# SMLC-NYSBC/TARGET-VAE

Measured on AMD Instinct MI355X. Metric: training images/sec (fwd+bwd+Adam), P8 z=2 64x64 bs=256/GPU, higher is better.
Workload: dtype f32 (matrix products: operands as TWO fp16 parts under one power-of-two scale PER ROW of the operand (row / column of the product), 3 fp16 MFMAs per product block -- 2 where one operand is the exact 0 / 1 matrix -- fp32 accumulate: at least as accurate against fp64 as the fp32 matrix pipe (profiles/

## Files before the change

### include/tvae_hip.h

```cpp
#ifndef TVAE_HIP_H
#define TVAE_HIP_H
#ifdef __cplusplus
extern "C" {
#endif

typedef void* tvae_stream_t;

int tvae_abi_version(void);


int tvae_rotate_bank_fwd(const float* weight, const int* tap_idx, const float* tap_w, float* bank, int C, int Cin,
                         int ksz, int R, tvae_stream_t stream);
int tvae_rotate_bank_bwd(const float* dbank, const int* csr_ptr, const int* csr_r, const int* csr_dst,
                         const float* csr_w, float* dweight, int C, int Cin, int ksz, int R, int accumulate,
                         tvae_stream_t stream);

int tvae_conv1_fwd(const float* y, const float* bank, const float* bias, float* out, int B, int Cin, int n, int ksz,
                   int pad, int C, int R, int act, float slope, tvae_stream_t stream);
int tvae_conv1_wgrad(const float* y, const float* dpre, float* dbank, float* ws, long ws_floats, int B, int Cin,
                     int n, int ksz, int pad, int C, int R, tvae_stream_t stream);

int tvae_linear_fwd(const float* W, const float* X, const float* bias, const float* gbias, int group,
                    const float* res, float* Y, int M, int N, int K, long ldx, long ldy, int act, float slope,
                    tvae_stream_t stream);
// ... 32 lines not shown
                       long ws_floats, int B, int Cin, int n, int ksz, int pad, int C, int R, int act, float slope,
                       int parts, tvae_stream_t stream);
int tvae_conv1_wgrad_dft(const float* dpre, const float* at, float* dbank, float* dbias, float* ws, long ws_floats, int B,
                         int Cin, int n, int ksz, int pad, int C, int R, int parts, tvae_stream_t stream);

long tvae_dense_x6_bytes(int rows, int K);
int tvae_dense_split3(const float* W, long ldw, void* a3, long a3_bytes, int rows, int K, int transpose,
                      const float* scale, float* rowsum, tvae_stream_t stream);
int tvae_dense_split2h(const float* W, long ldw, void* a3, long a3_bytes, int rows, int K, int transpose,
                       const float* scale, float* rowsum, tvae_stream_t stream);
int tvae_linear_fwd_x6(const void* w3, const float* X, const float* bias, const float* res, float* Y, int M, int N,
                       int K, long ldx, long ldy, int act, float slope, const float* col_w, const float* col_b,
                       float* col_y, const float* va_xr, const float* va_wc, const float* va_bc, const float* va_lb,
                       int va_np, void* sign_bits, int parts, const float* x_amax, float* y_amax, tvae_stream_t stream);
int tvae_linear_dgrad_x6(const void* w3t, const float* dpre, const float* add, const float* aux, float* dX, int M,
                         int N, int K, long ldd, long ldx, int mask, float slope, const float* in_xr,
                         const float* in_wc, float* in_gxr, float* in_part, long in_part_floats, const float* vg_wo,
                         const float* vg_gy, const float* vg_csum, const float* in_bc, const float* in_lb, int in_np,
                         float* rs_part, long rs_part_floats, const float* rs_wo, const float* rs_gysum, float* rs_db,
                         float* rs_dwo, int parts, const void* vg_bits, const float* rs_rowdot, const float* rs_bias,
                         const float* x_amax, float* y_amax, tvae_stream_t stream);
int tvae_dgrad_rowsum_total(const float* rs_part, int ntiles, int M, const float* rs_wo, const float* rs_gysum, float slope,
                            float* rs_db, float* rs_dwo, const float* rs_rowdot, const float* rs_bias, tvae_stream_t stream);
int tvae_dec_in_total(float* part, int B, int cpi, int F, float* Simg, float* dbc, float* dWc, tvae_stream_t stream);
long tvae_linear_wgrad_x6_ws_floats(int M, int N, int K);
int tvae_linear_wgrad_x6(const float* dpre, const float* X, float* dW, float* ws, long ws_floats, int M, int N, int K,
                         long ldd, long ldx, int accumulate, const float* vg_wo, const float* vg_gy, int vg_act,
                         float vg_slope, const float* va_xr, const float* va_wc, const float* va_bc, const float* va_lb,
                         int va_np, const void* vg_bits, int parts, const float* rd_w, long rd_ldw, float* rd_rowdot,
                         const float* a_amax, const float* x_amax, int x_amax_rows, tvae_stream_t stream);

int tvae_dec_out_bwd(const float* gy, int n_out, const float* Wo, const float* H, long ldh, float* D, long ldd, int F,
                     long N, int act, float slope, float* part, long part_floats, float* tot, tvae_stream_t stream);
int tvae_dec_in_bwd(const float* d, long ldd, const float* xr, const float* Wc, int F, int B, int Np, float* gxr,
                    float* Simg, float* dbc, float* dWc, float* part, long part_floats, tvae_stream_t stream);
int tvae_heads_fwd(const float* W, const float* X, long ldx, const float* bias, float* Y, long ldy, int nh, int C,
                   long N, tvae_stream_t stream);
int tvae_heads_bwd(const float* W, const float* dY, long ldy, const float* X, long ldx, float* dX, long lddx, int nh,
                   int C, long N, int act, float slope, float* part, long part_floats, float* tot,
                   tvae_stream_t stream);

int tvae_attn_head_fwd(const float* heads, long ldh, const float* E, const float* eps_z, const float* eps_t,
                       const float* p_r, const float* off, const float* p_tr, const float* grid, int B, int R, int P,
                       int zd, float sigma_p, float theta_off_scale, float* attn, float* q, float* a, float* z,
                       float* theta, float* dx, float* kl, float* part, long part_floats, tvae_stream_t stream);
int tvae_attn_head_bwd(const float* heads, long ldh, const float* q, const float* a, const float* eps_z,
// ... 75 lines not shown
```

### profiles/kernel_bench.py

```python
import os, sys, time
ROOT = os.path.dirname(os.path.dirname(os.path.abspath(__file__)))
sys.path[:0] = [ROOT, os.path.join(ROOT, 'target-vae_amd')]
import torch
import tvae._lib as _L
if os.environ.get('TVAE_LIB'):
    _L.LIB_PATH = os.path.abspath(os.environ['TVAE_LIB'])
from tvae._lib import call, set_gemm_mode, query
set_gemm_mode(os.environ.get('MODE', 'f32'))
print('mode', os.environ.get('MODE', 'f32'))
dev = torch.device('cuda:0')
reps = int(os.environ.get('REPS', '5'))
PARTS = int(os.environ.get('PARTS', '3'))
B = int(os.environ.get('B', '256'))
only = os.environ.get('ONLY', '')


def timeit(name, flops, fn):
    if only and not any(tok in name for tok in only.split(',')):
        return
    fn(); torch.cuda.synchronize()
    s, e = torch.cuda.Event(True), torch.cuda.Event(True)
    s.record()
    for _ in range(reps):
        fn()
# ... 83 lines not shown
    gxr = torch.empty(Nt, 2, device=dev); partf = torch.empty((Nt // 128) * F_ * 3, device=dev)
    wo1 = torch.randn(F_, device=dev); gy1 = torch.randn(Nt, device=dev)
    fl = 2.0 * F_ * F_ * Nt
    timeit('tail_dgrad_plain', fl, lambda: call('tvae_linear_dgrad_x6', w3t, h1, None, h3, h2, F_, Nt, F_, Nt, Nt, 1, 0.01, None, None, None, None, 0, None, None, None, None, None, 0, None, 0, None, None, None, None, PARTS))
    timeit('tail_dgrad_intail', fl, lambda: call('tvae_linear_dgrad_x6', w3t, h1, None, h3, None, F_, Nt, F_, Nt, Nt, 1, 0.01, xr2, wc2, gxr, partf, partf.numel(), None, None, None, None, None, 0, None, 0, None, None, None, None, PARTS))
    timeit('tail_dgrad_virt', fl, lambda: call('tvae_linear_dgrad_x6', w3t, h1, None, h3, h2, F_, Nt, F_, Nt, Nt, 1, 0.01, None, None, None, None, 0, wo1, gy1, None, None, None, 0, None, 0, None, None, None, None, PARTS))
    timeit('tail_dgrad_both', fl, lambda: call('tvae_linear_dgrad_x6', w3t, h1, None, h3, None, F_, Nt, F_, Nt, Nt, 1, 0.01, xr2, wc2, gxr, partf, partf.numel(), wo1, gy1, None, None, None, 0, None, 0, None, None, None, None, PARTS))
    timeit('tail_wgrad_plain', fl, lambda: call('tvae_linear_wgrad_x6', h1, h3, dW, ws, ws.numel(), F_, Nt, F_, Nt, Nt, 0, None, None, 0, 0.01, None, None, None, None, 0, None, PARTS))
    Np_ = n * n
    bc2 = torch.randn(F_, device=dev); lb2 = torch.randn(B, F_, device=dev)
    va = (xr2, wc2, bc2, lb2, Np_)
    cy = torch.empty(Nt, device=dev)
    timeit('tail_fwd_step', fl, lambda: call('tvae_linear_fwd_x6', w3, None, bb, None, h2, F_, Nt, F_, Nt, Nt, 1, 0.01, wo1, bb[:1].contiguous(), cy, *va, None, PARTS))
    sb = torch.zeros(F_, Nt // 32, dtype=torch.int32, device=dev)
    timeit('tail_fwd_step+bits', fl, lambda: call('tvae_linear_fwd_x6', w3, None, bb, None, h2, F_, Nt, F_, Nt, Nt, 1, 0.01, wo1, bb[:1].contiguous(), cy, *va, sb, PARTS))
    timeit('tail_fwd_step_nostore', fl, lambda: call('tvae_linear_fwd_x6', w3, None, bb, None, None, F_, Nt, F_, Nt, Nt, 1, 0.01, wo1, bb[:1].contiguous(), cy, *va, None, PARTS))
    csum2 = torch.empty(F_, device=dev)
    w3s = torch.empty_like(w3)
    call('tvae_dense_split3', W, F_, w3s, w3s.numel() * 4, F_, F_, 1, wo1, csum2)
    timeit('tail_dgrad_step', fl, lambda: call('tvae_linear_dgrad_x6', w3s, h1, None, None, None, F_, Nt, F_, Nt, Nt, 1, 0.01, xr2, wc2, gxr, partf, partf.numel(), None, gy1, csum2, bc2, lb2, Np_, None, 0, None, None, None, None, PARTS))
    timeit('tail_dgrad_generic', fl, lambda: call('tvae_linear_dgrad_x6', w3t, h1, None, None, None, F_, Nt, F_, Nt, Nt, 1, 0.01, xr2, wc2, gxr, partf, partf.numel(), wo1, gy1, None, bc2, lb2, Np_, None, 0, None, None, None, None, PARTS))
    hbits = torch.zeros(F_, Nt // 32, dtype=torch.int32, device=dev).random_(-2 ** 31, 2 ** 31 - 1)
    timeit('tail_wgrad_step', fl, lambda: call('tvae_linear_wgrad_x6', None, None, dW, ws, ws.numel(), F_, Nt, F_, Nt, Nt, 0, wo1, gy1, 1, 0.01, *va, hbits, PARTS))
    timeit('tail_wgrad_from_H', fl, lambda: call('tvae_linear_wgrad_x6', h1, None, dW, ws, ws.numel(), F_, Nt, F_, Nt, Nt, 0, wo1, gy1, 1, 0.01, *va, None, PARTS))
    timeit('tail_wgrad_virt', fl, lambda: call('tvae_linear_wgrad_x6', h1, h3, dW, ws, ws.numel(), F_, Nt, F_, Nt, Nt, 0, wo1, gy1, 1, 0.01, None, None, None, None, 0, None, PARTS))
if only and 'enc' in only:
    nh = 7
    Wh = torch.randn(nh, C, device=dev) * 0.1
    bh = torch.randn(nh, device=dev)
    heads = torch.empty(nh, N, device=dev)
    A1.normal_()
    fl2 = 2.0 * C * C * N
    timeit('enc_conv2_fwd_f32', fl2, lambda: call('tvae_linear_fwd', W2, A1, b2, None, 1, None, H, C, N, C, N, N, 1, 0.01))
    timeit('enc_heads_fwd', 2.0 * nh * C * N, lambda: call('tvae_heads_fwd', Wh, H, N, bh, heads, N, nh, C, N))
    w23 = torch.empty(query('tvae_dense_x6_bytes', C, C) // 4, device=dev)
    call('tvae_dense_split3', W2, C, w23, w23.numel() * 4, C, C, 0, None, None)
    H2 = torch.empty(C, N, device=dev)
    heads2 = torch.empty(nh, N, device=dev)
    timeit('enc_tail_fwd_x6', fl2, lambda: call('tvae_enc_tail_fwd_x6', w23, A1, N, b2, Wh, bh, nh, H2, N, heads2, N, None, None, C, N, 1, 0.01, PARTS))
    bits = torch.zeros(2, N, 4, dtype=torch.int32, device=dev)
    timeit('enc_tail_fwd_x6+bits', fl2, lambda: call('tvae_enc_tail_fwd_x6', w23, A1, N, b2, Wh, bh, nh, H2, N, heads2, N, bits[0], bits[1], C, N, 1, 0.01, PARTS))
    print('fused fwd vs separate: H %.3e heads %.3e' % (float((H2 - H).norm() / H.norm()), float((heads2 - heads).norm() / heads.norm())))
    dheads = torch.randn(nh, N, device=dev)
    dH = torch.empty(C, N, device=dev)
    npan = (N + 511) // 512
    part = torch.empty(npan * C * (nh + 1), device=dev)
# ... 14 lines not shown
```

### target-vae_amd/csrc/abi_dense_x6.hip

```cpp
#include "abi_dense_x6.hpp"
#include "dense_prepass_kernels.hpp"

using namespace tvae;

namespace {
struct Dx6Instance {
    int xv, epi, parts;
    int (*launch)(TVAE_DX6_LAUNCH_ARGS);
};
const Dx6Instance DX6_INSTANCES[] = {
#define TVAE_DX6(XV_, E_, NP_) {XV_, E_, NP_, dense_x6_launch<XV_, E_, NP_>},
#include "dense_x6_instances.def"
#undef TVAE_DX6
};
int dense_x6_dispatch(int xv, int epi, int parts, TVAE_DX6_LAUNCH_ARGS) {
    for (const Dx6Instance& i : DX6_INSTANCES)
        if (i.xv == xv && i.epi == epi && i.parts == parts)
            return i.launch(a3, X, ldx, ep, M, Mpad, N, K, K8pad, tm, bt, cd, it, vg, va, st, hs);
    return (int)hipErrorInvalidValue;
}
}

namespace tvae {
int h3_zero_slots(float* p, int n, int threads, hipStream_t st) {
// ... 78 lines not shown
    *rc = (int)hipGetLastError();
    return true;
}
}

namespace {
__global__ void dgrad_rowsum_total_kernel(const float* __restrict__ part, int ntiles, int K, const float* __restrict__ wo,
                                          const float* __restrict__ gysum, float slope, float* __restrict__ db,
                                          float* __restrict__ dwo, const float* __restrict__ rowdot,
                                          const float* __restrict__ bias) {
    __shared__ float sm[2 * 16];
    const int m = blockIdx.x;
    float s[2] = {0.f, 0.f};
    for (int t = threadIdx.x; t < ntiles; t += blockDim.x) {
        const float2 v = *reinterpret_cast<const float2*>(part + ((long)m * ntiles + t) * 2);
        s[0] += v.x;
        if (!rowdot) s[1] += v.y;
    }
    block_sum<2>(s, sm);
    if (threadIdx.x == 0) {
        const float g0 = __fmaf_rn(1.f - slope, s[0], slope * gysum[0]);
        db[m] = wo[m] * g0;
        dwo[m] = rowdot ? __fmaf_rn(bias ? bias[m] : 0.f, g0, rowdot[m]) : s[1];
    }
}
}

extern "C" {

long tvae_dense_x6_bytes(int rows, int K) { return dense_x6_bytes(rows, K); }
static int dense_split(const float* W, long ldw, void* a3, long a3_bytes, int rows, int K, int transpose,
                       const float* scale, float* rowsum, int parts, tvae_stream_t stream) {
    if (rows <= 0 || K <= 0) return 0;
    if (a3_bytes < tvae_dense_x6_bytes(rows, K) || !aligned16(a3)) return (int)hipErrorInvalidValue;
    const int Rpad = x6_round_up(rows, DX6_ROWS), K8pad = dense_k8pad(K);
    const long total = (long)K8pad * Rpad;
    if (parts == 2) {
        float* tr = h3_trailer(a3, rows, K);
        if (transpose)
            hipLaunchKernelGGL(dense_rowmax_kernel, dim3(Rpad / 64), dim3(1024), 0, S(stream), W, ldw, rows, Rpad, K, transpose,
                               scale, tr);
        else
            hipLaunchKernelGGL(dense_rowmax_rows_kernel, dim3(Rpad / 4), dim3(256), 0, S(stream), W, ldw, rows, Rpad, K, scale, tr);
        TVAE_CHECK_LAUNCH();
        const int rc = dense_split2h(W, ldw, (uint4*)a3, rows, Rpad, K, K8pad, transpose, scale, tr, S(stream));
        if (rc) return rc;
// ... 112 lines not shown
    if (in_xr) {
        if (!in_wc || !in_gxr || !in_part || in_part_floats < (long)(N / 128) * K * 3) return (int)hipErrorInvalidValue;
    } else if (!dX) {
        return (int)hipErrorInvalidValue;
    }
    if (vg_bits && !(vg_csum && rs_part && (rs_rowdot || !rs_db) && N % 32 == 0))
        return (int)hipErrorInvalidValue;
    if (rs_rowdot && !vg_bits) return (int)hipErrorInvalidValue;
    if (rs_part) {
        if (!vg_csum || !vg_gy || !rs_wo || !rs_gysum || (!rs_db != !rs_dwo) || M > DX6_ROWS || N % 128 != 0 ||
            rs_part_floats < (long)(N / 128) * M * 2 || (reinterpret_cast<size_t>(rs_part) & 7))
            return (int)hipErrorInvalidValue;
    }
    int rc = launch_dense_x6(w3t, dpre, ldd, ep, K, N, M, parts, S(stream), ColDot{nullptr, nullptr, nullptr},
                             InTail{in_xr, in_wc, in_gxr, in_part, in_bc, in_lb, in_np > 0 ? in_np : 1},
                             VirtGrad{vg_wo, vg_gy, mask, slope, vg_csum, (const unsigned*)vg_bits, rs_part, 0},
                             VirtAct{nullptr, nullptr, nullptr, nullptr, 1, 0, 0.f}, x_amax);
    if (rc || !rs_part || !rs_db || N <= 0 || K <= 0) return rc;
    hipLaunchKernelGGL(dgrad_rowsum_total_kernel, dim3(M), dim3(256), 0, S(stream), (const float*)rs_part, N / 128, M, rs_wo,
                       rs_gysum, slope, rs_db, rs_dwo, rs_rowdot, rs_bias);
    TVAE_CHECK_LAUNCH();
    return 0;
}
int tvae_dgrad_rowsum_total(const float* rs_part, int ntiles, int M, const float* rs_wo, const float* rs_gysum, float slope,
                            float* rs_db, float* rs_dwo, const float* rs_rowdot, const float* rs_bias, tvae_stream_t stream) {
    if (!rs_part || !rs_wo || !rs_gysum || !rs_db || !rs_dwo || ntiles <= 0 || M <= 0) return (int)hipErrorInvalidValue;
    hipLaunchKernelGGL(dgrad_rowsum_total_kernel, dim3(M), dim3(256), 0, S(stream), rs_part, ntiles, M, rs_wo, rs_gysum, slope,
                       rs_db, rs_dwo, rs_rowdot, rs_bias);
    TVAE_CHECK_LAUNCH();
    return 0;
}


}
```

### target-vae_amd/csrc/abi_dense_x6.hpp

```cpp
#pragma once
#include "abi_common.hpp"
#include "dense_x6_kernels.hpp"

namespace tvae {

static inline int dense_k8pad(int K) { return x6_round_up((K + 7) / 8, 2); }
static inline long dense_x6_bytes(int rows, int K) {
    const long Rpad = x6_round_up(rows, DX6_ROWS), K8pad = dense_k8pad(K);
    return 3 * K8pad * Rpad * 16;
}

static inline bool dense_x6_xres_fits(int rows_per_problem, int Mb, int N, int K, int parts) {
    const int nk = dense_k8pad(K) / 2;
    const size_t lds = (size_t)nk * parts * 256 * 16 + (size_t)(Mb + 128) * 4;
    return (parts == 2 || parts == 3) && (nk == 12 || nk == 10 || nk == 8) && N % 128 == 0 && rows_per_problem % DX6_ROWS == 0 &&
           Mb >= rows_per_problem && lds <= X6_LDS_MAX;
}

static inline float* h3_trailer(const void* a3, int rows, int K) {
    const long total = (long)dense_k8pad(K) * x6_round_up(rows, DX6_ROWS);
    return reinterpret_cast<float*>(const_cast<void*>(a3)) + 2 * total * 4;
}

#define TVAE_DX6_LAUNCH_ARGS                                                                                          \
    const uint4 *a3, const float *X, long ldx, const Epilogue &ep, int M, int Mpad, int N, int K, int K8pad,          \
        const TileMap &tm, const DenseBatch &bt, const ColDot &cd, const InTail &it, const VirtGrad &vg,              \
        const VirtAct &va, hipStream_t st, const H3Scale &hs
template <int XV, int EPI, int NP>
TVAE_INTERNAL int dense_x6_launch(TVAE_DX6_LAUNCH_ARGS);

#define TVAE_WG_LAUNCH_ARGS                                                                                           \
    int variant, const float *dY, long ldd, const float *X, long ldx, float *ws, int M, int Kf, int N, int nchunk,     \
        const TileMap &tm, const DenseBatch &bt, long dy_stride, const VirtGrad &vg, const VirtAct &va,               \
        const ATile &atile, hipStream_t st, const H3Scale &hs
TVAE_INTERNAL int dense_wgrad_x6_launch_p3(TVAE_WG_LAUNCH_ARGS);
TVAE_INTERNAL int dense_wgrad_x6_launch_p2(TVAE_WG_LAUNCH_ARGS);
TVAE_INTERNAL int dense_wgrad_x6_launch_p1(TVAE_WG_LAUNCH_ARGS);
TVAE_INTERNAL int dense_wgrad_x6_launch_p1_abf(TVAE_WG_LAUNCH_ARGS);

#define TVAE_WGW_LAUNCH_ARGS                                                                                          \
    const float *dY, long ldd, const float *X, long ldx, float *ws, int M, int Kf, int N, int nchunk, const TileMap &tm, \
        const DenseBatch &bt, long dy_stride, const ATile &atile, hipStream_t st, const H3Scale &hs
TVAE_INTERNAL int dense_wgrad_x6_wide_p3(TVAE_WGW_LAUNCH_ARGS);
TVAE_INTERNAL int dense_wgrad_x6_wide_p2(TVAE_WGW_LAUNCH_ARGS);

TVAE_INTERNAL int h3_zero_slots(float* p, int n, int threads, hipStream_t st);
TVAE_INTERNAL int dense_split2h(const float* W, long ldw, uint4* a3, int rows, int Rpad, int K, int K8pad, int transpose,
                                const float* scale, const float* rowmax, hipStream_t st);
TVAE_INTERNAL int dec_l0_bound(const float* xr, int N, const float* wc, const float* bc, const float* lb, long nlb, int K,
                               float* slots, hipStream_t st);

TVAE_INTERNAL int dense_x6_batched4(const void* w3, const float* X, long ldx, const Epilogue& ep, int rows_per_problem,
// ... 15 lines not shown
```

### target-vae_amd/csrc/dense_x6_kernels.hpp

```cpp
#pragma once
#include <hip/hip_runtime.h>
#include <type_traits>
#include "conv_x6_device.hpp"
#include "small_device.hpp"

#ifndef TVAE_ABL
#define TVAE_ABL 0
#endif

namespace tvae {

template <int NP>
__device__ __forceinline__ void mfma_np(f32x16& acc, const Cell16 (&a)[3], const Cell16 (&b)[3]) {
    if (NP == 3) mfma6(acc, a, b);
    else if (NP == 2) mfma3h(acc, a, b);
    else acc = __builtin_amdgcn_mfma_f32_32x32x16_bf16(a[0].v, b[0].v, acc, 0, 0, 0);
}
template <int NP>
__device__ __forceinline__ void mfma_part(f32x16& acc, const Cell16& a, const Cell16& b) {
    if (NP == 2) acc = __builtin_amdgcn_mfma_f32_32x32x16_f16(a.h, b.h, acc, 0, 0, 0);
    else acc = __builtin_amdgcn_mfma_f32_32x32x16_bf16(a.v, b.v, acc, 0, 0, 0);
}
template <int NP> struct OneBits { static constexpr unsigned lo = NP == 2 ? 0x3c00u : 0x3f80u, hi = lo << 16; };
template <bool XS>
// ... 204 lines not shown
#pragma unroll
                for (int j = 0; j < 4; ++j) {
                    float v = NP == 2 ? __fmaf_rn(acc[i][j][r] * ixv[j], aq[p], bq[p]) : acc[i][j][r] + bq[p];
                    v = fmaxf(v, v * slope);
                    ysum[j] = __fmaf_rn(wq[p], v, ysum[j]);
                    const unsigned long long bl = __ballot(v > 0.f);
                    sw[j] = (unsigned)(half ? bl >> 32 : bl);
                }
                if ((lane & 31) == 0 && sbits)
                    *reinterpret_cast<uint4*>(sbits + (long)(m0 + rb + p) * bitw + (n0 >> 5)) = make_uint4(sw[0], sw[1], sw[2], sw[3]);
            }
            __builtin_amdgcn_sched_barrier(0);
        }
}

__device__ __forceinline__ float half_wave_sum_hi(float x) {
    x = dpp_add<0xB1>(x);
    x = dpp_add<0x4E>(x);
    x = dpp_add<0x141>(x);
    x = dpp_add<0x140>(x);
    return x + __int_as_float(__builtin_amdgcn_update_dpp(0, __float_as_int(x), 0x142, 0xA, 0xF, false));
}

template <int NP>
__device__ __forceinline__ void dense_x6_epilogue_lean_in(f32x16 (&acc)[2][4], const float* bsm, const float* wc2,
                                                          const float* cbm, const float* h3a, float slope, float oms, int wave,
                                                          int lane, int m0, int M, int tile_n, const float (&gyv)[4],
                                                          const float (&x0)[4], const float (&x1)[4], float* part,
                                                          float (&gsum)[4][2]) {
    float gx0[4], gx1[4];
#pragma unroll
    for (int j = 0; j < 4; ++j) {
        gx0[j] = gyv[j] * x0[j];
        gx1[j] = gyv[j] * x1[j];
    }
    const int half = lane >> 5;
#pragma unroll
    for (int i = 0; i < 2; ++i)
#pragma unroll
        for (int q = 0; q < 4; ++q) {
            const int rb = wave * 64 + i * 32 + 8 * q + 4 * half;
            const float4 b4 = *reinterpret_cast<const float4*>(bsm + rb);
            const float4 c4 = *reinterpret_cast<const float4*>(cbm + rb);
            const float4 l4 = *reinterpret_cast<const float4*>(cbm + DX6_ROWS + rb);
            const float4 wA = *reinterpret_cast<const float4*>(wc2 + 2 * rb), wB = *reinterpret_cast<const float4*>(wc2 + 2 * rb + 4);
            float4 a4 = make_float4(1.f, 1.f, 1.f, 1.f);
            if (NP == 2) a4 = *reinterpret_cast<const float4*>(h3a + rb);
            const float bq[4] = {b4.x, b4.y, b4.z, b4.w}, cq[4] = {c4.x, c4.y, c4.z, c4.w}, lq[4] = {l4.x, l4.y, l4.z, l4.w};
            const float aq[4] = {a4.x, a4.y, a4.z, a4.w};
            const float w0q[4] = {wA.x, wA.z, wB.x, wB.z}, w1q[4] = {wA.y, wA.w, wB.y, wB.w};
#pragma unroll
            for (int p = 0; p < 4; ++p) {
                const int r = 4 * q + p;
                float rs0 = 0.f, rs1 = 0.f, rs2 = 0.f;
#pragma unroll
                for (int j = 0; j < 4; ++j) {
                    const float t = __fmaf_rn(oms, NP == 2 ? acc[i][j][r] * aq[p] : acc[i][j][r], bq[p]);
                    const float pre = dec_l0_pre(w0q[p], w1q[p], cq[p], lq[p], x0[j], x1[j]);
                    const float u = pre > 0.f ? t : t * slope;
                    rs0 = __fmaf_rn(u, gyv[j], rs0);
                    rs1 = __fmaf_rn(u, gx0[j], rs1);
                    rs2 = __fmaf_rn(u, gx1[j], rs2);
                    gsum[j][0] = __fmaf_rn(w0q[p], u, gsum[j][0]);
                    gsum[j][1] = __fmaf_rn(w1q[p], u, gsum[j][1]);
                }
                rs0 = half_wave_sum_hi(rs0);
                rs1 = half_wave_sum_hi(rs1);
// ... 1380 lines not shown
```

### target-vae_amd/tvae/_lib.py

```python
from __future__ import annotations

import ctypes
import os

import torch

_HERE = os.path.dirname(os.path.abspath(__file__))
LIB_PATH = os.environ.get('TVAE_LIB') or os.path.join(os.path.dirname(_HERE), 'csrc', 'build', 'libtvae_hip.so')

SIGNATURES = {
    'tvae_rotate_bank_fwd': 'ppppiiii',
    'tvae_rotate_bank_bwd': 'ppppppiiiii',
    'tvae_conv1_fwd': 'ppppiiiiiiiif',
    'tvae_conv1_wgrad': 'ppppl iiiiiii'.replace(' ', ''),
    'tvae_bank_split3': 'ppliiii',
    'tvae_conv1_fwd_x6': 'ppppiiiiiiiif',
    'tvae_dy_split3': 'ppliiiiiii',
    'tvae_conv1_wgrad_x6': 'ppppliiiiiii',
    'tvae_conv1_fwd_dft': 'ppppppliiiiiiiifi',
    'tvae_conv1_wgrad_dft': 'pppppliiiiiiii',
    'tvae_dense_split3': 'plpliiipp',
    'tvae_dense_split2h': 'plpliiipp',
    'tvae_linear_fwd_x6': 'pppppiiillifpppppppipipp',
    'tvae_linear_dgrad_x6': 'pppppiiillifpppplpppppiplppppippppp',
    'tvae_dec_in_total': 'piiippp',
    'tvae_dgrad_rowsum_total': 'piippfpppp',
    'tvae_linear_wgrad_x6': 'ppppliiillippifppppipiplpppi',
    'tvae_linear_fwd': 'ppppippiiillif',
    'tvae_linear_dgrad': 'pppppiiillif',
    'tvae_linear_wgrad': 'ppppliiilli',
    'tvae_rowdot_seg': 'plpiiiipp',
    'tvae_seg_sum': 'pilpfi',
    'tvae_coldot': 'pliipiipip',
    'tvae_outer_mask': 'pipiiplpliiif',
    'tvae_act_bwd': 'ppplif',
    'tvae_dec_out_bwd': 'pipplplilifplp',
    'tvae_dec_in_bwd': 'plppiiipppppl',
    'tvae_heads_fwd': 'pplppliil',
    'tvae_heads_bwd': 'pplplpliilifplp',
    'tvae_attn_head_fwd': 'plpppppppiiiiffppppppppl',
    'tvae_attn_head_bwd': 'plppppppppiiiiffpppppppppl',
    'tvae_get_latent': 'plpppiiiifppp',
    'tvae_enc_tail_fwd_x6': 'pplpppiplplppilifip',
    'tvae_enc_tail_dgrad_x6': 'ppplippplilfi',
    'tvae_enc_tail_wgrad_x6': 'plplipppplilfip',
    'tvae_enc_tail_fwd_wide': 'ppplppiplplppilifip',
    'tvae_enc_tail_dgrad_wide': 'ppplippplplilfip',
# ... 11 lines not shown
    'tvae_loglik_bwd': 'ppppiii',
    'tvae_elbo_reduce': 'ppippp',
    'tvae_elbo_reduce_bwd': 'pppipp',
    'tvae_ctf_corr': 'pppiiii',
    'tvae_loglik_masked_fwd': 'pppffiip',
    'tvae_loglik_masked_bwd': 'pppffiipp',
    'tvae_adam_flat': 'pppplfffffff',
}

QUERIES = {
    'tvae_conv1_x6_supported': ('iiii', 'i'),
    'tvae_conv1_x6_bank_bytes': ('iiii', 'l'),
    'tvae_conv1_x6_dy_bytes': ('iiiiii', 'l'),
    'tvae_dense_x6_bytes': ('ii', 'l'),
    'tvae_conv1_dft_supported': ('iiiiiii', 'i'),
    'tvae_conv1_dft_at_floats': ('iiiiiii', 'l'),
    'tvae_conv1_dft_ws_floats': ('iiiiiii', 'l'),
    'tvae_conv1_dft_frame': ('iiiiiii', 'i'),
    'tvae_conv1_dft_ring': ('iiiiiii', 'i'),
    'tvae_conv1_dft_route': ('iiiiiiiii', 'i'),
    'tvae_enc_tail_wgrad_x6_ws_floats': ('l', 'l'),
    'tvae_enc_tail_wide_max_rows': ('', 'i'),
    'tvae_linear_wgrad_x6_ws_floats': ('iii', 'l'),
}

OPTIONAL_TAIL = {'tvae_linear_wgrad_x6': 6}

_CT = {'p': ctypes.c_void_p, 'i': ctypes.c_int, 'l': ctypes.c_long, 'f': ctypes.c_float}
_lib = None


class TvaeHipError(RuntimeError):
    pass


def lib():
    global _lib
    if _lib is None:
        if not os.path.exists(LIB_PATH):
            raise TvaeHipError(
                f'{LIB_PATH} not found: build it with `make -C target-vae_amd/csrc` '
                '(or __graft_entry__.build()).  There is no CPU fallback.')
        L = ctypes.CDLL(LIB_PATH)
        for name, sig in SIGNATURES.items():
            fn = getattr(L, name)
            fn.restype = ctypes.c_int
# ... 198 lines not shown
```

### target-vae_amd/tvae/ops.py

```python
from __future__ import annotations

import math
import os
from typing import NamedTuple, Optional

import numpy as np
import torch

from . import tables
from ._lib import arithmetic, call, get_gemm_mode, parts, query, split_pipe

ACT_NONE, ACT_LRELU, ACT_TANH = 0, 1, 2
LRELU_SLOPE = 0.01


def _expect(cond: bool, what: str) -> None:
    if not cond:
        raise ValueError('tvae.ops: ' + what)


def act_code(activation) -> int:
    import torch.nn as nn
    a = activation() if isinstance(activation, type) else activation
    if isinstance(a, nn.LeakyReLU):
# ... 688 lines not shown

    @staticmethod
    def forward(ctx, xc, dx, theta):
        B, Np = theta.shape[0], xc.shape[0]
        _expect(tuple(xc.shape) == (Np, 2) and tuple(dx.shape) == (B, 2) and theta.dim() == 1, 'coordinate shapes')
        xc, dx, theta = xc.contiguous(), dx.contiguous(), theta.contiguous()
        xr = torch.empty(B, Np, 2, dtype=torch.float32, device=xc.device)
        call('tvae_coord_fwd', xc, dx, theta, xr, B, Np)
        ctx.save_for_backward(xc, dx, theta)
        return xr

    @staticmethod
    def backward(ctx, g):
        xc, dx, theta = ctx.saved_tensors
        B, Np = theta.shape[0], xc.shape[0]
        gdx = torch.empty(B, 2, dtype=torch.float32, device=xc.device)
        gth = torch.empty(B, dtype=torch.float32, device=xc.device)
        call('tvae_coord_bwd', xc, dx, theta, g.contiguous(), gdx, gth, B, Np)
        return None, gdx, gth


DEC_PAD = os.environ.get('TVAE_DEC_PAD', '1') != '0'
DEC_LD_PAD = int(os.environ.get('TVAE_DEC_LD_PAD', '64'))


class DecoderRoute(NamedTuple):
    ldn: int
    split: bool
    four_x6: bool
    four_dgrad_x6: bool
    virt_act: bool
    fused_out: bool
    virt_grad: bool
    sign_bits: bool
    no_h: bool
    h3: bool
    infer: bool


def decoder_route(B: int, Np: int, F_: int, n_hidden: int, n_out: int, act: int, resid: bool, Ff: int,
                  infer: bool) -> DecoderRoute:
    Nt = B * Np
    split = _dense_x6_ok(F_, Nt)
    virt_grad = n_hidden >= 1 and n_out == 1 and not resid and split
    sign_bits = virt_grad and act == ACT_LRELU
    ld_pad = DEC_LD_PAD and (Ff or n_hidden >= 2) and Nt % 16384 == 0 and split
# ... 197 lines not shown
                xb = xb * gy_amax()
            wg = _wgrad(dsrc, hprev, F_, Nt, F_, vg if use_vg else None, va, act, sbits, rowdot_w=W if from_bits else None,
                        a_amax=d_bnd if plain_h3 else None, x_amax=xb, ld=ldn)
            dW, rowdot = wg if from_bits else (wg, None)
            db = drow if drow is not None else _rowsum(d, F_, Nt, ld=ldn)
            drow = None
            fuse_in = li == 0 and rt.virt_act
            dprev = None if fuse_in else torch.empty(F_, ldn, dtype=torch.float32, device=dev)
            if rt.split:
                two_val = use_vg and act == ACT_LRELU
                p_d = 2 if (rt.h3 and (two_val or (not use_vg and d_bnd is not None))) else _p3()
                if p_d == 2 and not two_val:
                    _note('dec.dgrad_h3_meas')
                emit = dmeas[li:li + 1] if (dmeas is not None and not fuse_in) else None
                if two_val:
                    w3t, csum = _split_weight(W, F_, F_, True, 'x6_dense_wt', scale=vg[0], nparts=p_d)
                    _note('dec.virt_grad_2val')
                else:
                    w3t, csum = _split_weight(W, F_, F_, True, 'x6_dense_wt', nparts=p_d), None
                if fuse_in:
                    gxr_f = torch.empty(B, Np, 2, dtype=torch.float32, device=dev)
                    part_f = workspace(dev, (Nt // 128) * F_ * 3)
                rs_part = _scratch(dev, 'dec_rs_part', (Nt // 128) * F_ * 2) if from_bits else None
                with _timed('tvae_linear_dgrad_x6', p_d, two_val):
                    call('tvae_linear_dgrad_x6', w3t, dsrc, d if resid else None, hprev, dprev, F_, Nt, F_, ldn, ldn, act,
                         LRELU_SLOPE, xr.view(Nt, 2) if fuse_in else None, Wc.contiguous() if fuse_in else None,
                         gxr_f if fuse_in else None, part_f if fuse_in else None, part_f.numel() if fuse_in else 0,
                         vg[0] if (use_vg and not two_val) else None, vg[1] if use_vg else None, csum,
                         bc if va else None, LB if va else None, Np if va else 0,
                         rs_part, rs_part.numel() if from_bits else 0, vg[0] if from_bits else None,
                         dbo if from_bits else None, tot[0] if from_bits else None, tot[1] if from_bits else None, p_d,
                         sbits if from_bits else None, rowdot, b if from_bits else None,
                         d_bnd if (p_d == 2 and not two_val) else None, emit)
                if fuse_in:
                    _note('dec.fuse_in')
                d_bnd = emit
                if two_val and li == 0 and has_f and rt.h3:
                    d_bnd = gy_amax() * (W.detach().abs() * vg[0].detach().abs()[:, None]).sum(0).amax().reshape(1)
            else:
                call('tvae_linear_dgrad', W.contiguous(), d, d if resid else None, hprev, dprev, F_, Nt, F_, ldn, ldn,
                     act, LRELU_SLOPE)
            d = dprev
            grads_hidden.append((dW, db))
        grads_hidden.reverse()
        Simg = torch.empty(B, F_, dtype=torch.float32, device=dev)
        dbc = torch.empty(F_, dtype=torch.float32, device=dev)
        gxr = gxr_f if rt.virt_act else torch.empty(B, Np, 2, dtype=torch.float32, device=dev)
        if rt.virt_act:
            dWc = torch.empty(F_, 2, dtype=torch.float32, device=dev)
            call('tvae_dec_in_total', part_f, B, Np // 128, F_, Simg, dbc, dWc)
        elif has_f:
            call('tvae_rowdot_seg', d, ldn, None, 1, F_, Nt, Np, Simg)
            call('tvae_seg_sum', Simg, B, F_, dbc, 1.0, 0)
        else:
            dWc = torch.empty(F_, 2, dtype=torch.float32, device=dev)
            part = workspace(dev, B * ((Np + 1023) // 1024) * F_ * 3)
# ... 142 lines not shown
```

Baseline: 27940.

## Add half-row-tile dgrad kernel for fused decoder input layer with 2-part weights

Adds a specialized dgrad kernel for the decoder's first hidden layer when the virtual-gradient is two-valued and rebuilt from sign bits. Each block covers 256 of the 512 rows instead of the full height, which doubles the grid and raises the occupancy target to two blocks per CU. The partial input-gradient sums go to a 5-slot workspace, and a new total kernel reduces them alongside the row-sum bias/weight reduction. The cost is an extra workspace round trip and a narrow route that only fires for F=512 without residual connections.

```diff
diff --git a/include/tvae_hip.h b/include/tvae_hip.h
--- a/include/tvae_hip.h
+++ b/include/tvae_hip.h
@@ -78,6 +78,13 @@
                          const float* x_amax, float* y_amax, tvae_stream_t stream);
 int tvae_dgrad_rowsum_total(const float* rs_part, int ntiles, int M, const float* rs_wo, const float* rs_gysum, float slope,
                             float* rs_db, float* rs_dwo, const float* rs_rowdot, const float* rs_bias, tvae_stream_t stream);
+long tvae_linear_dgrad_x6_half_ws_floats(int N);
+int tvae_linear_dgrad_x6_half(const void* w3t, int M, int N, int K, float slope, const float* in_xr, const float* in_wc,
+                              float* in_gxr, float* in_part, long in_part_floats, const float* vg_gy, const float* vg_csum,
+                              const float* in_bc, const float* in_lb, int in_np, float* rs_part, long rs_part_floats,
+                              const float* rs_wo, const float* rs_gysum, float* rs_db, float* rs_dwo, int parts,
+                              const void* vg_bits, const float* rs_rowdot, const float* rs_bias, float* gws, long gws_floats,
+                              tvae_stream_t stream);
 int tvae_dec_in_total(float* part, int B, int cpi, int F, float* Simg, float* dbc, float* dWc, tvae_stream_t stream);
 long tvae_linear_wgrad_x6_ws_floats(int M, int N, int K);
 int tvae_linear_wgrad_x6(const float* dpre, const float* X, float* dW, float* ws, long ws_floats, int M, int N, int K,
diff --git a/profiles/kernel_bench.py b/profiles/kernel_bench.py
--- a/profiles/kernel_bench.py
+++ b/profiles/kernel_bench.py
@@ -129,6 +129,17 @@
     timeit('tail_dgrad_generic', fl, lambda: call('tvae_linear_dgrad_x6', w3t, h1, None, None, None, F_, Nt, F_, Nt, Nt, 1, 0.01, xr2, wc2, gxr, partf, partf.numel(), wo1, gy1, None, bc2, lb2, Np_, None, 0, None, None, None, None, PARTS))
     hbits = torch.zeros(F_, Nt // 32, dtype=torch.int32, device=dev).random_(-2 ** 31, 2 ** 31 - 1)
     timeit('tail_wgrad_step', fl, lambda: call('tvae_linear_wgrad_x6', None, None, dW, ws, ws.numel(), F_, Nt, F_, Nt, Nt, 0, wo1, gy1, 1, 0.01, *va, hbits, PARTS))
+    if PARTS == 2:
+        from tvae.ops import DGRAD_HALF
+        w3h = torch.empty_like(w3)
+        call('tvae_dense_split2h', W, F_, w3h, w3h.numel() * 4, F_, F_, 1, wo1, csum2)
+        rsp = torch.empty((Nt // 128) * F_ * 2, device=dev); gys = gy1.sum().reshape(1)
+        rdb, rdwo, rdot = torch.empty(F_, device=dev), torch.empty(F_, device=dev), torch.randn(F_, device=dev)
+        if DGRAD_HALF:
+            gws = torch.empty(query('tvae_linear_dgrad_x6_half_ws_floats', Nt), device=dev)
+            timeit('tail_dgrad_step_bits_half', fl, lambda: call('tvae_linear_dgrad_x6_half', w3h, F_, Nt, F_, 0.01, xr2, wc2, gxr, partf, partf.numel(), gy1, csum2, bc2, lb2, Np_, rsp, rsp.numel(), wo1, gys, rdb, rdwo, 2, hbits, rdot, bb, gws, gws.numel()))
+        else:
+            timeit('tail_dgrad_step_bits', fl, lambda: call('tvae_linear_dgrad_x6', w3h, None, None, None, None, F_, Nt, F_, Nt, Nt, 1, 0.01, xr2, wc2, gxr, partf, partf.numel(), None, gy1, csum2, bc2, lb2, Np_, rsp, rsp.numel(), wo1, gys, rdb, rdwo, 2, hbits, rdot, bb))
     timeit('tail_wgrad_from_H', fl, lambda: call('tvae_linear_wgrad_x6', h1, None, dW, ws, ws.numel(), F_, Nt, F_, Nt, Nt, 0, wo1, gy1, 1, 0.01, *va, None, PARTS))
     timeit('tail_wgrad_virt', fl, lambda: call('tvae_linear_wgrad_x6', h1, h3, dW, ws, ws.numel(), F_, Nt, F_, Nt, Nt, 0, wo1, gy1, 1, 0.01, None, None, None, None, 0, None, PARTS))
 if only and 'enc' in only:
diff --git a/target-vae_amd/csrc/abi_dense_x6.hip b/target-vae_amd/csrc/abi_dense_x6.hip
--- a/target-vae_amd/csrc/abi_dense_x6.hip
+++ b/target-vae_amd/csrc/abi_dense_x6.hip
@@ -1,5 +1,6 @@
 #include "abi_dense_x6.hpp"
 #include "dense_prepass_kernels.hpp"
+#include "dense_x6_half_shape.hpp"
 
 using namespace tvae;
 
@@ -124,6 +125,37 @@
         const float g0 = __fmaf_rn(1.f - slope, s[0], slope * gysum[0]);
         db[m] = wo[m] * g0;
         dwo[m] = rowdot ? __fmaf_rn(bias ? bias[m] : 0.f, g0, rowdot[m]) : s[1];
+    }
+}
+__global__ void dgrad_half_total_kernel(const float* __restrict__ part, int ntiles, int M, const float* __restrict__ wo,
+                                        const float* __restrict__ gysum, float slope, float* __restrict__ db,
+                                        float* __restrict__ dwo, const float* __restrict__ rowdot,
+                                        const float* __restrict__ bias, const float4* __restrict__ gws,
+                                        float4* __restrict__ gxr, long n4) {
+    __shared__ float sm[16];
+    if ((int)blockIdx.x >= M) {
+        const long i = (long)(blockIdx.x - M) * blockDim.x + threadIdx.x;
+        if (i >= n4) return;
+        float4 g = gws[i];
+#pragma unroll
+        for (int w = 1; w < 5; ++w) {
+            const float4 c = gws[w * n4 + i];
+            g.x += c.x;
+            g.y += c.y;
+            g.z += c.z;
+            g.w += c.w;
+        }
+        gxr[i] = g;
+        return;
+    }
+    const int m = blockIdx.x;
+    float s[1] = {0.f};
+    for (int t = threadIdx.x; t < ntiles; t += blockDim.x) s[0] += part[((long)m * ntiles + t) * 2];
+    block_sum<1>(s, sm);
+    if (threadIdx.x == 0) {
+        const float g0 = __fmaf_rn(1.f - slope, s[0], slope * gysum[0]);
+        db[m] = wo[m] * g0;
+        dwo[m] = __fmaf_rn(bias ? bias[m] : 0.f, g0, rowdot[m]);
     }
 }
 }
@@ -282,6 +314,40 @@
     TVAE_CHECK_LAUNCH();
     return 0;
 }
+long tvae_linear_dgrad_x6_half_ws_floats(int N) { return N > 0 ? (long)DXH_GWS_SLOTS * 2 * N : 0; }
+int tvae_linear_dgrad_x6_half(const void* w3t, int M, int N, int K, float slope, const float* in_xr, const float* in_wc,
+                              float* in_gxr, float* in_part, long in_part_floats, const float* vg_gy, const float* vg_csum,
+                              const float* in_bc, const float* in_lb, int in_np, float* rs_part, long rs_part_floats,
+                              const float* rs_wo, const float* rs_gysum, float* rs_db, float* rs_dwo, int parts,
+                              const void* vg_bits, const float* rs_rowdot, const float* rs_bias, float* gws, long gws_floats,
+                              tvae_stream_t stream) {
+    if (K != DX6_ROWS || M <= 0 || M > DXH_KMAX || N <= 0 || N % 128 != 0 || parts != 2 || in_np <= 0 || in_np % 128 != 0)
+        return (int)hipErrorInvalidValue;
+    if (!w3t || !in_xr || !in_wc || !in_gxr || !in_part || !vg_gy || !vg_csum || !in_bc || !rs_part || !rs_wo || !rs_gysum ||
+        !rs_db || !rs_dwo || !vg_bits || !rs_rowdot || !gws)
+        return (int)hipErrorInvalidValue;
+    if (in_part_floats < (long)(N / 128) * K * 3 || rs_part_floats < (long)(N / 128) * M * 2 ||
+        gws_floats < tvae_linear_dgrad_x6_half_ws_floats(N))
+        return (int)hipErrorInvalidValue;
+    if (!aligned16(w3t) || !aligned16(vg_bits) || !aligned16(gws) || !aligned16(in_gxr) || (reinterpret_cast<size_t>(rs_part) & 7))
+        return (int)hipErrorInvalidValue;
+    TileMap tm{DX6_ROWS / DXH_ROWS, N / 128, 1};
+    tm.pack = 1;
+    H3Scale hs = H3_NONE;
+    hs.amax_a = h3_trailer(w3t, K, M);
+    hs.a_rows = 1;
+    int rc = dense_x6_half_launch_p2((const uint4*)w3t, slope, K, DX6_ROWS, N, M, dense_k8pad(M), tm,
+                                     InTail{in_xr, in_wc, in_gxr, in_part, in_bc, in_lb, in_np},
+                                     VirtGrad{nullptr, vg_gy, ACT_LRELU, slope, vg_csum, (const unsigned*)vg_bits, rs_part, 0}, hs,
+                                     gws, S(stream));
+    if (rc) return rc;
+    const long n4 = (long)N / 2;
+    hipLaunchKernelGGL(dgrad_half_total_kernel, dim3((unsigned)(M + (n4 + 255) / 256)), dim3(256), 0, S(stream),
+                       (const float*)rs_part, N / 128, M, rs_wo, rs_gysum, slope, rs_db, rs_dwo, rs_rowdot, rs_bias,
+                       (const float4*)gws, (float4*)in_gxr, n4);
+    TVAE_CHECK_LAUNCH();
+    return 0;
+}
 int tvae_dgrad_rowsum_total(const float* rs_part, int ntiles, int M, const float* rs_wo, const float* rs_gysum, float slope,
                             float* rs_db, float* rs_dwo, const float* rs_rowdot, const float* rs_bias, tvae_stream_t stream) {
     if (!rs_part || !rs_wo || !rs_gysum || !rs_db || !rs_dwo || ntiles <= 0 || M <= 0) return (int)hipErrorInvalidValue;
diff --git a/target-vae_amd/csrc/abi_dense_x6.hpp b/target-vae_amd/csrc/abi_dense_x6.hpp
--- a/target-vae_amd/csrc/abi_dense_x6.hpp
+++ b/target-vae_amd/csrc/abi_dense_x6.hpp
@@ -28,6 +28,11 @@
         const VirtAct &va, hipStream_t st, const H3Scale &hs
 template <int XV, int EPI, int NP>
 TVAE_INTERNAL int dense_x6_launch(TVAE_DX6_LAUNCH_ARGS);
+
+#define TVAE_DXH_LAUNCH_ARGS                                                                                          \
+    const uint4 *a3, float slope, int M, int Mpad, int N, int K, int K8pad, const TileMap &tm, const InTail &it,      \
+        const VirtGrad &vg, const H3Scale &hs, float *gws, hipStream_t st
+TVAE_INTERNAL int dense_x6_half_launch_p2(TVAE_DXH_LAUNCH_ARGS);
 
 #define TVAE_WG_LAUNCH_ARGS                                                                                           \
     int variant, const float *dY, long ldd, const float *X, long ldx, float *ws, int M, int Kf, int N, int nchunk,     \
diff --git a/target-vae_amd/csrc/dense_x6_half_instance.hip b/target-vae_amd/csrc/dense_x6_half_instance.hip
--- /dev/null
+++ b/target-vae_amd/csrc/dense_x6_half_instance.hip
@@ -0,0 +1,12 @@
+#include "abi_dense_x6.hpp"
+#include "dense_x6_half_kernels.hpp"
+
+namespace tvae {
+#define TVAE_DXH_PASTE_(a, b) a##b
+#define TVAE_DXH_PASTE(a, b) TVAE_DXH_PASTE_(a, b)
+int TVAE_DXH_PASTE(dense_x6_half_launch_p, TVAE_DXH_NP)(TVAE_DXH_LAUNCH_ARGS) {
+    hipLaunchKernelGGL((dense_x6_half_kernel<TVAE_DXH_NP>), dim3(tm.grid()), dim3(DXH_THREADS), 0, st, a3, slope, M, Mpad, N, K,
+                       K8pad, tm, it, vg, hs, gws);
+    return (int)hipGetLastError();
+}
+}
diff --git a/target-vae_amd/csrc/dense_x6_half_kernels.hpp b/target-vae_amd/csrc/dense_x6_half_kernels.hpp
--- /dev/null
+++ b/target-vae_amd/csrc/dense_x6_half_kernels.hpp
@@ -0,0 +1,171 @@
+#pragma once
+#include "dense_x6_kernels.hpp"
+#include "dense_x6_half_shape.hpp"
+
+namespace tvae {
+
+template <int NP>
+static __global__ __launch_bounds__(DXH_THREADS, 2)
+void dense_x6_half_kernel(const uint4* __restrict__ A3, float slope, int M, int Mpad, int N, int K, int K8pad, TileMap tm,
+                          InTail it, VirtGrad vg, H3Scale hs, float* __restrict__ gws) {
+    __shared__ __attribute__((aligned(16))) uint4 Bs[2 * 2 * 128];
+    __shared__ __attribute__((aligned(16))) unsigned wbits[4 * DXH_KMAX];
+    __shared__ __attribute__((aligned(16))) float bsm[DXH_ROWS];
+    __shared__ __attribute__((aligned(16))) float wsm_[2 * DXH_ROWS];
+    __shared__ __attribute__((aligned(16))) float cbm_[2 * DXH_ROWS];
+    __shared__ __attribute__((aligned(16))) float h3a_[NP == 2 ? DXH_ROWS : 4];
+    __shared__ float rsm_[2 * DXH_KMAX + 4];
+    const int tid = threadIdx.x, lane = tid & 63;
+    const int wave = __builtin_amdgcn_readfirstlane(tid >> 6);
+    int tile_m, tile_n, split_unused;
+    if (!tm.decode(blockIdx.x, tile_m, tile_n, split_unused)) return;
+    const int m0 = tile_m * DXH_ROWS, n0 = tile_n * 128;
+    const int khalf = lane >> 5;
+    const int nk = K8pad >> 1;
+    if (NP == 2) h3a_[tid] = h3_inv(h3_scale(hs.amax_a[m0 + tid]));
+    bsm[tid] = vg.slope * vg.csum[m0 + tid];
+    wsm_[2 * tid] = it.wc[2 * (m0 + tid)];
+    wsm_[2 * tid + 1] = it.wc[2 * (m0 + tid) + 1];
+    {
+        const int img_ = n0 / it.Np;
+        cbm_[tid] = it.bc[m0 + tid];
+        cbm_[DXH_ROWS + tid] = it.lb ? it.lb[(long)img_ * M + m0 + tid] : 0.f;
+    }
+    {
+        const long bitw = (long)(N >> 5);
+        const unsigned* brow = vg.bits + (n0 >> 5);
+#pragma unroll
+        for (int h = 0; h < DXH_KMAX / DXH_THREADS; ++h) {
+            const int k = tid + h * DXH_THREADS;
+            uint4 w = make_uint4(0u, 0u, 0u, 0u);
+            if (k < K) w = *reinterpret_cast<const uint4*>(brow + (long)k * bitw);
+            wbits[k] = w.x;
+            wbits[DXH_KMAX + k] = w.y;
+            wbits[2 * DXH_KMAX + k] = w.z;
+            wbits[3 * DXH_KMAX + k] = w.w;
+        }
+    }
+
+    const long part_cells = (long)K8pad * Mpad;
+    const uint4* a_ptr = A3 + (long)khalf * Mpad + m0 + 64 * wave + (lane & 31);
+    auto load_a = [&](int t, Cell16 (&a)[2][3]) {
+        const uint4* q = a_ptr + (long)(2 * t) * Mpad;
+#pragma unroll
+        for (int i = 0; i < 2; ++i)
+#pragma unroll
+            for (int p = 0; p < NP; ++p) a[i][p].u = q[p * part_cells + i * 32];
+    };
+    const int kq = tid >> 7, nb = tid & 127;
+    const float vg_g = vg.gy[n0 + nb];
+    const unsigned* wcol = wbits + (nb >> 5) * DXH_KMAX + 4 * kq;
+    const int sh = nb & 31;
+    auto load_x = [&](int t, uint4 (&x)[2]) {
+#pragma unroll
+        for (int h = 0; h < 2; ++h) x[h] = *reinterpret_cast<const uint4*>(wcol + 16 * t + 8 * h);
+    };
+    auto store_b = [&](int stage, const uint4 (&x)[2]) {
+#pragma unroll
+        for (int h = 0; h < 2; ++h) {
+            uint2* dst = reinterpret_cast<uint2*>(Bs + stage * 256 + h * 128 + nb) + kq;
+            const bool p0 = (x[h].x >> sh) & 1u, p1 = (x[h].y >> sh) & 1u, p2 = (x[h].z >> sh) & 1u, p3 = (x[h].w >> sh) & 1u;
+            dst[0] = make_uint2((p0 ? OneBits<NP>::lo : 0u) | (p1 ? OneBits<NP>::hi : 0u),
+                                (p2 ? OneBits<NP>::lo : 0u) | (p3 ? OneBits<NP>::hi : 0u));
+        }
+    };
+    auto row_sums = [&](int t, bool real, const uint4 (&x)[2]) {
+        const uint4 xs = tile_m ? x[1] : x[0];
+        const int slot = real ? (wave & 1) * DXH_KMAX + ((16 * t + 4 * (kq + 2 * tile_m)) & (DXH_KMAX - 1)) : 2 * DXH_KMAX;
+        const float a[4] = {((xs.x >> sh) & 1u) ? vg_g : 0.f, ((xs.y >> sh) & 1u) ? vg_g : 0.f,
+                            ((xs.z >> sh) & 1u) ? vg_g : 0.f, ((xs.w >> sh) & 1u) ? vg_g : 0.f};
+        const float tot = wave_sum4(a, lane);
+        if (lane < 4) rsm_[slot + lane] = tot;
+    };
+
+    f32x16 acc[2][4];
+#pragma unroll
+    for (int i = 0; i < 2; ++i)
+#pragma unroll
+        for (int j = 0; j < 4; ++j)
+#pragma unroll
+            for (int r = 0; r < 16; ++r) acc[i][j][r] = 0.f;
+
+    Cell16 afA[2][3], afB[2][3];
+    uint4 xA[2], xB[2];
+    __syncthreads();
+    {
+        uint4 x0[2];
+        load_x(0, x0);
+        load_a(0, afA);
+        load_x(nk > 1 ? 1 : 0, xB);
+        store_b(0, x0);
+        row_sums(0, true, x0);
+    }
+    __syncthreads();
+    auto step = [&](int t, Cell16 (&afc)[2][3], Cell16 (&afn)[2][3], uint4 (&xn)[2], uint4 (&xf)[2]) {
+        const int cur = t & 1;
+        load_a(t + 1 < nk ? t + 1 : t, afn);
+        load_x(t + 2 < nk ? t + 2 : t, xf);
+        const uint4* bs = Bs + cur * 256 + khalf * 128 + (lane & 31);
+#pragma unroll
+        for (int j = 0; j < 4; ++j) {
+            Cell16 b0;
+            b0.u = bs[j * 32];
+#pragma unroll
+            for (int i = 0; i < 2; ++i)
+#pragma unroll
+                for (int p = 0; p < NP; ++p) mfma_part<NP>(acc[i][j], afc[i][p], b0);
+            if (j == 1) {
+                store_b(cur ^ 1, xn);
+                row_sums(t + 1, t + 1 < nk, xn);
+            }
+        }
+        __builtin_amdgcn_sched_barrier(0);
+        __syncthreads();
+    };
+    int tt = 0;
+    for (; tt + 1 < nk; tt += 2) {
+        step(tt, afA, afB, xB, xA);
+        step(tt + 1, afB, afA, xA, xB);
+    }
+    if (nk & 1) step(nk - 1, afA, afB, xB, xA);
+    {
+#pragma unroll
+        for (int h = 0; h < DXH_KMAX / DXH_THREADS; ++h) {
+            const int k = tid + h * DXH_THREADS;
+            if (k < K && ((k >> 3) & 1) == tile_m) vg.rpart[((long)k * (N >> 7) + tile_n) * 2] = rsm_[k] + rsm_[DXH_KMAX + k];
+        }
+    }
+    float gsum[4][2] = {{0.f, 0.f}, {0.f, 0.f}, {0.f, 0.f}, {0.f, 0.f}};
+    float gyv[4], x0_[4], x1_[4];
+#pragma unroll
+    for (int j = 0; j < 4; ++j) {
+        const long nn = n0 + j * 32 + (lane & 31);
+        gyv[j] = vg.gy[nn];
+        x0_[j] = it.xr[2 * nn];
+        x1_[j] = it.xr[2 * nn + 1];
+    }
+    dense_x6_epilogue_lean_in<NP, DXH_ROWS>(acc, bsm, wsm_, cbm_, h3a_, slope, 1.f - vg.slope, wave, lane, m0, M, tile_n, gyv, x0_,
+                                            x1_, it.part, gsum);
+    float* cds = reinterpret_cast<float*>(Bs);
+#pragma unroll
+    for (int j = 0; j < 4; ++j)
+#pragma unroll
+        for (int k = 0; k < 2; ++k) {
+            const float v = gsum[j][k] + __shfl_xor(gsum[j][k], 32, 64);
+            if (lane < 32) cds[(wave * 128 + j * 32 + lane) * 2 + k] = v;
+        }
+    __syncthreads();
+    float* g = gws + 2 * (long)n0 + tid;
+    const long gslot = 2 * (long)N;
+    if (tile_m == 0) {
+        float s = 0.f;
+#pragma unroll
+        for (int w = 0; w < 4; ++w) s += cds[w * 256 + tid];
+        g[0] = s;
+    } else {
+#pragma unroll
+        for (int w = 0; w < 4; ++w) g[(1 + w) * gslot] = cds[w * 256 + tid];
+    }
+}
+
+}
diff --git a/target-vae_amd/csrc/dense_x6_half_shape.hpp b/target-vae_amd/csrc/dense_x6_half_shape.hpp
--- /dev/null
+++ b/target-vae_amd/csrc/dense_x6_half_shape.hpp
@@ -0,0 +1,10 @@
+#pragma once
+
+namespace tvae {
+
+constexpr int DXH_THREADS = 256;
+constexpr int DXH_ROWS = 256;
+constexpr int DXH_KMAX = 512;
+constexpr int DXH_GWS_SLOTS = 5;
+
+}
diff --git a/target-vae_amd/csrc/dense_x6_kernels.hpp b/target-vae_amd/csrc/dense_x6_kernels.hpp
--- a/target-vae_amd/csrc/dense_x6_kernels.hpp
+++ b/target-vae_amd/csrc/dense_x6_kernels.hpp
@@ -250,7 +250,7 @@
     return x + __int_as_float(__builtin_amdgcn_update_dpp(0, __float_as_int(x), 0x142, 0xA, 0xF, false));
 }
 
-template <int NP>
+template <int NP, int ROWS = DX6_ROWS>
 __device__ __forceinline__ void dense_x6_epilogue_lean_in(f32x16 (&acc)[2][4], const float* bsm, const float* wc2,
                                                           const float* cbm, const float* h3a, float slope, float oms, int wave,
                                                           int lane, int m0, int M, int tile_n, const float (&gyv)[4],
@@ -270,7 +270,7 @@
             const int rb = wave * 64 + i * 32 + 8 * q + 4 * half;
             const float4 b4 = *reinterpret_cast<const float4*>(bsm + rb);
             const float4 c4 = *reinterpret_cast<const float4*>(cbm + rb);
-            const float4 l4 = *reinterpret_cast<const float4*>(cbm + DX6_ROWS + rb);
+            const float4 l4 = *reinterpret_cast<const float4*>(cbm + ROWS + rb);
             const float4 wA = *reinterpret_cast<const float4*>(wc2 + 2 * rb), wB = *reinterpret_cast<const float4*>(wc2 + 2 * rb + 4);
             float4 a4 = make_float4(1.f, 1.f, 1.f, 1.f);
             if (NP == 2) a4 = *reinterpret_cast<const float4*>(h3a + rb);
diff --git a/target-vae_amd/tvae/_lib.py b/target-vae_amd/tvae/_lib.py
--- a/target-vae_amd/tvae/_lib.py
+++ b/target-vae_amd/tvae/_lib.py
@@ -23,6 +23,7 @@
     'tvae_dense_split2h': 'plpliiipp',
     'tvae_linear_fwd_x6': 'pppppiiillifpppppppipipp',
     'tvae_linear_dgrad_x6': 'pppppiiillifpppplpppppiplppppippppp',
+    'tvae_linear_dgrad_x6_half': 'piiifpppplppppiplppppippppl',
     'tvae_dec_in_total': 'piiippp',
     'tvae_dgrad_rowsum_total': 'piippfpppp',
     'tvae_linear_wgrad_x6': 'ppppliiillippifppppipiplpppi',
@@ -80,6 +81,7 @@
     'tvae_enc_tail_wgrad_x6_ws_floats': ('l', 'l'),
     'tvae_enc_tail_wide_max_rows': ('', 'i'),
     'tvae_linear_wgrad_x6_ws_floats': ('iii', 'l'),
+    'tvae_linear_dgrad_x6_half_ws_floats': ('i', 'l'),
 }
 
 OPTIONAL_TAIL = {'tvae_linear_wgrad_x6': 6}
diff --git a/target-vae_amd/tvae/ops.py b/target-vae_amd/tvae/ops.py
--- a/target-vae_amd/tvae/ops.py
+++ b/target-vae_amd/tvae/ops.py
@@ -734,6 +734,7 @@
 
 DEC_PAD = os.environ.get('TVAE_DEC_PAD', '1') != '0'
 DEC_LD_PAD = int(os.environ.get('TVAE_DEC_LD_PAD', '64'))
+DGRAD_HALF = os.environ.get('TVAE_DGRAD_HALF', '1') != '0'
 
 
 class DecoderRoute(NamedTuple):
@@ -977,16 +978,25 @@
                     gxr_f = torch.empty(B, Np, 2, dtype=torch.float32, device=dev)
                     part_f = workspace(dev, (Nt // 128) * F_ * 3)
                 rs_part = _scratch(dev, 'dec_rs_part', (Nt // 128) * F_ * 2) if from_bits else None
+                half = (DGRAD_HALF and two_val and from_bits and fuse_in and va is not None and p_d == 2 and F_ == 512 and
+                        not resid and Nt % 128 == 0 and Np % 128 == 0)
                 with _timed('tvae_linear_dgrad_x6', p_d, two_val):
-                    call('tvae_linear_dgrad_x6', w3t, dsrc, d if resid else None, hprev, dprev, F_, Nt, F_, ldn, ldn, act,
-                         LRELU_SLOPE, xr.view(Nt, 2) if fuse_in else None, Wc.contiguous() if fuse_in else None,
-                         gxr_f if fuse_in else None, part_f if fuse_in else None, part_f.numel() if fuse_in else 0,
-                         vg[0] if (use_vg and not two_val) else None, vg[1] if use_vg else None, csum,
-                         bc if va else None, LB if va else None, Np if va else 0,
-                         rs_part, rs_part.numel() if from_bits else 0, vg[0] if from_bits else None,
-                         dbo if from_bits else None, tot[0] if from_bits else None, tot[1] if from_bits else None, p_d,
-                         sbits if from_bits else None, rowdot, b if from_bits else None,
-                         d_bnd if (p_d == 2 and not two_val) else None, emit)
+                    if half:
+                        _note('dec.dgrad_half')
+                        gws = _scratch(dev, 'dec_dgrad_half', query('tvae_linear_dgrad_x6_half_ws_floats', Nt))
+                        call('tvae_linear_dgrad_x6_half', w3t, F_, Nt, F_, LRELU_SLOPE, xr.view(Nt, 2), Wc.contiguous(), gxr_f,
+                             part_f, part_f.numel(), vg[1], csum, bc, LB, Np, rs_part, rs_part.numel(), vg[0], dbo, tot[0],
+                             tot[1], p_d, sbits, rowdot, b, gws, gws.numel())
+                    else:
+                        call('tvae_linear_dgrad_x6', w3t, dsrc, d if resid else None, hprev, dprev, F_, Nt, F_, ldn, ldn, act,
+                             LRELU_SLOPE, xr.view(Nt, 2) if fuse_in else None, Wc.contiguous() if fuse_in else None,
+                             gxr_f if fuse_in else None, part_f if fuse_in else None, part_f.numel() if fuse_in else 0,
+                             vg[0] if (use_vg and not two_val) else None, vg[1] if use_vg else None, csum,
+                             bc if va else None, LB if va else None, Np if va else 0,
+                             rs_part, rs_part.numel() if from_bits else 0, vg[0] if from_bits else None,
+                             dbo if from_bits else None, tot[0] if from_bits else None, tot[1] if from_bits else None, p_d,
+                             sbits if from_bits else None, rowdot, b if from_bits else None,
+                             d_bnd if (p_d == 2 and not two_val) else None, emit)
                 if fuse_in:
                     _note('dec.fuse_in')
                 d_bnd = emit
```

Result: no change. 27820 (-0.4%).
